# LemonATsu/DANBO-pytorch

Measured on AMD Instinct MI355X. Metric: ray-samples/sec at 512x512x64 samples, higher is better.
Workload: dtype f32 (fp16x2-split MFMA products, fp32 accumulate); 1 GPU; H36M danbo_base network, 512x512 rays x (48 coarse + 16 importance) samples, 1 pose / 1 camera per rank, cylinder near/far, exact in-volume culling; rays=262144, samples_per_ray=64, parallelism=rays-dp1

## Files before the change

danbo-pytorch_amd/csrc/common.hpp:

```cpp
#pragma once
#include <hip/hip_runtime.h>
#include <stdint.h>
#include <algorithm>
#include <atomic>
#include "../../include/danbo_hip.h"
#include "sample_math.hpp"

#define DANBO_CHECK_ARG(cond) do { if (!(cond)) return DANBO_EINVAL; } while (0)
#define DANBO_CHECK_DENSITY_ACT(act, shift) \
    DANBO_CHECK_ARG(((act) == DANBO_DENSITY_RELU || (act) == DANBO_DENSITY_SOFTPLUS) && (shift) - (shift) == 0.f)
static inline bool poses_ok(int R, int G) { return R > 0 && G > 0 && R % G == 0; }
static inline bool shape_ok(int R, int S, int G) { return S > 0 && poses_ok(R, G); }
static inline bool one_of(const void* z, const void* pts) { return (z == nullptr) != (pts == nullptr); }
#define DANBO_TRY(call) do { const int rc_ = (call); if (rc_ != 0) return rc_; } while (0)
#define DANBO_LAUNCH_RET() do { hipError_t e_ = hipGetLastError(); return e_ == hipSuccess ? 0 : (int)e_; } while (0)

#define DANBO_ENSURE_LDS(func, bytes)                                                                              \
    do {                                                                                                           \
        static std::atomic<unsigned long long> done_{0};                                                           \
        int dev_ = 0;                                                                                              \
        if (hipGetDevice(&dev_) != hipSuccess) return (int)hipGetLastError();                                      \
        const unsigned long long bit_ = 1ull << (dev_ & 63);                                                       \
        if (!(done_.load(std::memory_order_acquire) & bit_)) {                                                     \
            const hipError_t e_ = hipFuncSetAttribute(reinterpret_cast<const void*>(func),                         \
                                                      hipFuncAttributeMaxDynamicSharedMemorySize, (int)(bytes));   \
            if (e_ != hipSuccess) return (int)e_;                                                                  \
            done_.fetch_or(bit_, std::memory_order_release);                                                       \
        }                                                                                                          \
    } while (0)

#if defined(__HIP_DEVICE_COMPILE__)
#define DANBO_NO_PK_F32 __attribute__((target("no-packed-fp32-ops")))
#else
#define DANBO_NO_PK_F32
#endif

namespace danbo {

constexpr int WAVE = 64;
typedef _Float16 half8 __attribute__((ext_vector_type(8)));
typedef float f32x4 __attribute__((ext_vector_type(4)));
typedef float f32x16 __attribute__((ext_vector_type(16)));
typedef unsigned u32x4 __attribute__((ext_vector_type(4)));

#ifdef DANBO_DEV_SWITCHES
static inline int dev_env(const char* name, int dflt) { const char* e = getenv(name); return e ? atoi(e) : dflt; }
#else
static constexpr int dev_env(const char*, int dflt) { return dflt; }
#endif

static inline int num_cu() {
    static std::atomic<int> cached_[64];
    int dev = 0;
    if (hipGetDevice(&dev) != hipSuccess) return 256;
    std::atomic<int>& c = cached_[dev & 63];
    int n = c.load(std::memory_order_relaxed);
    if (n == 0) {
        if (hipDeviceGetAttribute(&n, hipDeviceAttributeMultiprocessorCount, dev) != hipSuccess || n <= 0) n = 256;
        { const int v = dev_env("DANBO_NUM_CU", 0); if (v > 0 && v <= n) n = v; }
        c.store(n, std::memory_order_relaxed);
    }
    return n;
}

struct Carver {
    char* base = nullptr;
    size_t used = 0;
    Carver() {}
    explicit Carver(void* workspace) : base(reinterpret_cast<char*>(((uintptr_t)workspace + 255) & ~(uintptr_t)255)) {}
    void align() { used = (used + 255) & ~(size_t)255; }
    template <class T>
    T* take(size_t n) {
        align();
        T* p = base ? reinterpret_cast<T*>(base + used) : nullptr;
        used += n * sizeof(T);
        return p;
    }
};

static inline int ceil_div(long a, long b) { return (int)((a + b - 1) / b); }

static inline int stream_grid(long items, int block) {
    long g = (items + block - 1) / block;
    const long cap = (long)num_cu() * 8;
    if (g > cap) g = cap;
    if (g < 1) g = 1;
    return (int)g;
}

template <class K>
static inline int resident_grid(K kernel, long items, int block, size_t lds = 0) {
    int per_cu = 0;
    if (hipOccupancyMaxActiveBlocksPerMultiprocessor(&per_cu, kernel, block, lds) != hipSuccess || per_cu < 1) per_cu = 1;
    long g = (items + block - 1) / block;
    const long cap = (long)num_cu() * per_cu;
    if (g > cap) g = cap;
    if (g < 1) g = 1;
    return (int)g;
}

__device__ __forceinline__ float wave_sum(float v) {
#pragma unroll
    for (int off = 32; off > 0; off >>= 1) v += __shfl_xor(v, off, 64);
    return v;
}

__device__ __forceinline__ void pe_sincos(float x, float* s, float* c) {
    const float k = rintf(x * 0.636619772367581343f);
    float r = fmaf(k, -1.57079601287841796875f, x);
    r = fmaf(k, -3.1391647326017846353352069854736328125e-7f, r);
    r = fmaf(k, -5.390302529957764765544681040410068817436695098876953125e-15f, r);
    const float r2 = r * r;
    float sp = fmaf(r2, 2.6083159809786593541502952575683593750e-6f, -1.981069071916863322258e-4f);
    sp = fmaf(sp, r2, 8.33307858556509017944e-3f);
    sp = fmaf(sp, r2, -1.66666597127914428711e-1f);
    const float sn = fmaf(sp * r2, r, r);
    float cp = fmaf(r2, 2.44331571593647822737693786621e-5f, -1.38873163610696792602539062500e-3f);
    cp = fmaf(cp, r2, 4.16666455566883087158203125e-2f);
    cp = fmaf(cp, r2, -0.5f);
    const float cs = fmaf(cp, r2, 1.0f);
    const int q = (int)k;
    const float s0 = (q & 1) ? cs : sn;
    const float c0 = (q & 1) ? sn : cs;
    *s = (q & 2) ? -s0 : s0;
    *c = ((q + 1) & 2) ? -c0 : c0;
}

#define DANBO_DPP_STEP(OP, IDENT, CTRL, ROWMASK)                                                              \
    {                                                                                                          \
        const int t_ = __builtin_amdgcn_update_dpp(__builtin_bit_cast(int, (float)(IDENT)),                    \
                                                   __builtin_bit_cast(int, x), CTRL, ROWMASK, 0xf, false);     \
        x = OP(x, __builtin_bit_cast(float, t_));                                                              \
    }
__device__ __forceinline__ float dpp_add_(float a, float b) { return add_rn(a, b); }
__device__ __forceinline__ float dpp_mul_(float a, float b) { return mul_rn(a, b); }

__device__ __forceinline__ float wave_scan_add(float x) {
    DANBO_DPP_STEP(dpp_add_, 0.f, 0x111, 0xf) DANBO_DPP_STEP(dpp_add_, 0.f, 0x112, 0xf)
    DANBO_DPP_STEP(dpp_add_, 0.f, 0x114, 0xf) DANBO_DPP_STEP(dpp_add_, 0.f, 0x118, 0xf)
    DANBO_DPP_STEP(dpp_add_, 0.f, 0x142, 0xa) DANBO_DPP_STEP(dpp_add_, 0.f, 0x143, 0xc)
    return x;
}
__device__ __forceinline__ float wave_scan_mul(float x) {
    DANBO_DPP_STEP(dpp_mul_, 1.f, 0x111, 0xf) DANBO_DPP_STEP(dpp_mul_, 1.f, 0x112, 0xf)
    DANBO_DPP_STEP(dpp_mul_, 1.f, 0x114, 0xf) DANBO_DPP_STEP(dpp_mul_, 1.f, 0x118, 0xf)
    DANBO_DPP_STEP(dpp_mul_, 1.f, 0x142, 0xa) DANBO_DPP_STEP(dpp_mul_, 1.f, 0x143, 0xc)
    return x;
}
__device__ __forceinline__ uint32_t wave_or(uint32_t x) {
#define DANBO_DPP_OR(CTRL, ROWMASK) x |= (uint32_t)__builtin_amdgcn_update_dpp(0, (int)x, CTRL, ROWMASK, 0xf, false);
    DANBO_DPP_OR(0x111, 0xf) DANBO_DPP_OR(0x112, 0xf) DANBO_DPP_OR(0x114, 0xf) DANBO_DPP_OR(0x118, 0xf)
    DANBO_DPP_OR(0x142, 0xa) DANBO_DPP_OR(0x143, 0xc)
#undef DANBO_DPP_OR
    return (uint32_t)__builtin_amdgcn_readlane((int)x, 63);
}
__device__ __forceinline__ float wave_total(float x) {
    return __builtin_bit_cast(float, __builtin_amdgcn_readlane(__builtin_bit_cast(int, wave_scan_add(x)), 63));
}

__device__ __forceinline__ float lane_xor32(float x) {
    const unsigned u = __builtin_bit_cast(unsigned, x);
    const auto r = __builtin_amdgcn_permlane32_swap(u, u, false, false);
    return __builtin_bit_cast(float, (threadIdx.x & 32) ? r[0] : r[1]);
}
__device__ __forceinline__ float lane_xor16(float x) {
    const unsigned u = __builtin_bit_cast(unsigned, x);
    const auto r = __builtin_amdgcn_permlane16_swap(u, u, false, false);
    return __builtin_bit_cast(float, (threadIdx.x & 16) ? r[0] : r[1]);
}

static __global__ __launch_bounds__(256) void k_zero_words_(uint32_t* __restrict__ p0, long n0, uint32_t* __restrict__ p1, long n1) {
    const long stride = (long)gridDim.x * blockDim.x;
    for (long i = (long)blockIdx.x * blockDim.x + threadIdx.x; i < n0; i += stride) p0[i] = 0u;
    for (long i = (long)blockIdx.x * blockDim.x + threadIdx.x; i < n1; i += stride) p1[i] = 0u;
}
static inline void zero_words(void* p0, long n0, void* p1, long n1, hipStream_t st) {
    const long n = n0 > n1 ? n0 : n1;
    hipLaunchKernelGGL(k_zero_words_, dim3(stream_grid(n, 256)), dim3(256), 0, st, static_cast<uint32_t*>(p0), n0,
                       static_cast<uint32_t*>(p1), p1 ? n1 : 0);
}
static __global__ __launch_bounds__(64) void k_copy_words_(const uint32_t* __restrict__ s0, uint32_t* __restrict__ d0, int n0,
                                                           const uint32_t* __restrict__ s1, uint32_t* __restrict__ d1, int n1) {
    for (int i = threadIdx.x; i < n0; i += 64) d0[i] = s0[i];
    for (int i = threadIdx.x; i < n1; i += 64) d1[i] = s1[i];
}

template <int BLOCK>
__device__ __forceinline__ void stage_bone_tables(const float* __restrict__ align, const float* __restrict__ axis_scale,
                                                  float* s_align, float* s_scale, float pad) {
    for (int i = threadIdx.x; i < J * 16; i += BLOCK) s_align[i] = align[i];
    for (int i = threadIdx.x; i < J * 4; i += BLOCK) s_scale[i] = (i & 3) < 3 ? fabsf(axis_scale[(i >> 2) * 3 + (i & 3)]) : pad;
}

__device__ __forceinline__ int resolve_count(const int32_t* count, int n_cap) {
    if (count == nullptr) return n_cap;
    int c = *count;
    return c < n_cap ? c : n_cap;
}

template <class H8>
__device__ __forceinline__ void split8_mix(const float* v, H8& hi, H8& lo) {
    u32x4 h, l;
#pragma unroll
    for (int p = 0; p < 4; ++p) {
        unsigned hp, lp;
        asm("v_cvt_pk_f16_f32 %0, %1, %2" : "=v"(hp) : "v"(v[2 * p]), "v"(v[2 * p + 1]));
        asm("v_fma_mixlo_f16 %0, %1, 1.0, -%2 op_sel:[0,0,0] op_sel_hi:[0,0,1]" : "=v"(lp) : "v"(v[2 * p]), "v"(hp));
        asm("v_fma_mixhi_f16 %0, %1, 1.0, -%2 op_sel:[0,0,1] op_sel_hi:[0,0,1]" : "+v"(lp) : "v"(v[2 * p + 1]), "v"(hp));
        h[p] = hp;
        l[p] = lp;
    }
    hi = __builtin_bit_cast(H8, h);
    lo = __builtin_bit_cast(H8, l);
}


}
```

danbo-pytorch_amd/csrc/k_sample.hip:

```cpp
#include "common.hpp"
#include "cull_math.hpp"

namespace danbo {

__global__ __launch_bounds__(256) DANBO_NO_PK_F32 void k_cylinder_pass1(const float* __restrict__ rays_o,
                                                        const float* __restrict__ rays_d,
                                                        const float* __restrict__ cyl, int R, int G,
                                                        float near0, float far0,
                                                        const float* __restrict__ near_in,
                                                        const float* __restrict__ far_in, int chunk,
                                                        double* __restrict__ acc,
                                                        float* __restrict__ near_out,
                                                        float* __restrict__ far_out) {
    const int rays_per_pose = R / G;
    for (int r0 = blockIdx.x * blockDim.x; r0 < R; r0 += gridDim.x * blockDim.x) {
        const int r = r0 + threadIdx.x;
        const bool act = r < R;
        const int rc = act ? r : R - 1;
        const int g = min(rc / rays_per_pose, G - 1);
        float o[3] = {rays_o[3 * rc], rays_o[3 * rc + 1], rays_o[3 * rc + 2]};
        float d[3] = {rays_d[3 * rc], rays_d[3 * rc + 1], rays_d[3 * rc + 2]};
        float c[3] = {cyl[5 * g], cyl[5 * g + 1], cyl[5 * g + 2]};
        float nr, fr;
        const bool hit = cylinder_bounds(o, d, c, near_in ? near_in[rc] : near0, far_in ? far_in[rc] : far0, &nr, &fr) && act;
// ... 378 lines not shown
            pa[0] = pts[3 * mac]; pa[1] = pts[3 * mac + 1]; pa[2] = pts[3 * mac + 2];
            pb[0] = pts[3 * mbc]; pb[1] = pts[3 * mbc + 1]; pb[2] = pts[3 * mbc + 2];
        } else {
            const float oa[3] = {rays_o[3 * ra], rays_o[3 * ra + 1], rays_o[3 * ra + 2]};
            const float da[3] = {rays_d[3 * ra], rays_d[3 * ra + 1], rays_d[3 * ra + 2]};
            const float ob[3] = {rays_o[3 * rb], rays_o[3 * rb + 1], rays_o[3 * rb + 2]};
            const float db[3] = {rays_d[3 * rb], rays_d[3 * rb + 1], rays_d[3 * rb + 2]};
            sample_point(oa, da, ma < M ? zreg[2 * pr] : z[M - 1], pa);
            sample_point(ob, db, mb < M ? zreg[2 * pr + 1] : z[M - 1], pb);
        }
        const int ga = pose_of(ra), gb = pose_of(rb);
        uint32_t ba = 0, bb = 0;
        uint32_t need = (1u << J) - 1u;
        if (ray_mask != nullptr) {
            need = wave_or(pre[2 * pr] | pre[2 * pr + 1]);
        } else if (prefilter) {
            uint32_t mine = s_mask[ra - r_first] | s_mask[rb - r_first];
            need = wave_or(mine);
        }
        if (__builtin_amdgcn_readfirstlane((int)__all(ga == gb))) {
            const v2f px = {pa[0], pb[0]}, py = {pa[1], pb[1]}, pz = {pa[2], pb[2]};
            const float* sk = s_skt + (ga - g0) * J * 16;
            in_volume_pk(sk, s_align, s_scale, need, px, py, pz, ba, bb);
        } else {
            const float* ska = s_skt + (ga - g0) * J * 16;
            const float* skb = s_skt + (gb - g0) * J * 16;
            for (int j = 0; j < J; ++j) {
                float pt[3];
                bone_local(ska + 16 * j, s_align + 16 * j, pa, pt);
                ba |= (in_volume(pt, s_scale + 4 * j) ? 1u : 0u) << j;
                bone_local(skb + 16 * j, s_align + 16 * j, pb, pt);
                bb |= (in_volume(pt, s_scale + 4 * j) ? 1u : 0u) << j;
            }
        }
        bits4[2 * pr] = ma < M ? ba : 0u;
        bits4[2 * pr + 1] = mb < M ? bb : 0u;
        if (ma < M) valid_bits[ma] = ba;
        if (mb < M) valid_bits[mb] = bb;
    }
    if (list != nullptr) {
        __shared__ int s_cnt[CULL_SPT * (CULL_BLOCK / 64)];
        __shared__ int s_base;
        const int wave = threadIdx.x >> 6;
        unsigned long long ball[CULL_SPT];
#pragma unroll
        for (int it = 0; it < CULL_SPT; ++it) {
            ball[it] = __ballot(bits4[it] != 0);
            if (lane == 0) s_cnt[it * (CULL_BLOCK / 64) + wave] = __popcll(ball[it]);
        }
        __syncthreads();
        if (threadIdx.x == 0) {
            int run = 0;
            for (int i = 0; i < CULL_SPT * (CULL_BLOCK / 64); ++i) { const int c = s_cnt[i]; s_cnt[i] = run; run += c; }
            s_base = run > 0 ? atomicAdd(count, run) : 0;
        }
        __syncthreads();
#pragma unroll
        for (int it = 0; it < CULL_SPT; ++it) {
            if (bits4[it] != 0) {
                const long m = base + it * CULL_BLOCK + threadIdx.x;
                list[s_base + s_cnt[it * (CULL_BLOCK / 64) + wave] + __popcll(ball[it] & ((1ull << lane) - 1ull))] = (int32_t)m;
            }
        }
    }
}

constexpr int GATHER_TS = 16;
constexpr int GATHER_BLOCK = GATHER_TS * J;

__global__ __launch_bounds__(GATHER_BLOCK) void k_bone_gather(const float* __restrict__ rays_o,
                                                              const float* __restrict__ rays_d,
                                                              const float* __restrict__ z,
                                                              const float* __restrict__ pts, int R, int S, int G,
                                                              const float* __restrict__ skts,
                                                              const float* __restrict__ align,
                                                              const float* __restrict__ axis_scale,
                                                              const float* __restrict__ volumes,
                                                              const int32_t* __restrict__ list,
                                                              const int32_t* __restrict__ count, int n_cap,
                                                              float* __restrict__ part_feat) {
    __shared__ __attribute__((aligned(16))) float s_vol[J * VOL];
    __shared__ __attribute__((aligned(16))) float s_out[GATHER_TS * J * FEAT];
    __shared__ __attribute__((aligned(16))) float s_skt[J * 16];
    __shared__ __attribute__((aligned(16))) float s_align[J * 16];
    __shared__ float s_scale[J * 4];

    const int n = resolve_count(count, n_cap);
    const int ntiles = (n + GATHER_TS - 1) / GATHER_TS;
    const long spp = (long)(R / G) * S;
    const int tid = threadIdx.x;
    const int sl = tid / J, j = tid % J;

    stage_bone_tables<GATHER_BLOCK>(align, axis_scale, s_align, s_scale, 1.f);
    int g_lds = -1;

    for (int tile = blockIdx.x; tile < ntiles; tile += gridDim.x) {
        const int row0 = tile * GATHER_TS;
        const int first = list ? list[row0] : row0;
        const int g_tile = pose_of_sample(first, spp, G);
        __syncthreads();
        if (g_tile != g_lds) {
            const float4* src = reinterpret_cast<const float4*>(volumes + (size_t)g_tile * J * VOL);
            float4* dst = reinterpret_cast<float4*>(s_vol);
            for (int i = tid; i < J * VOL / 4; i += GATHER_BLOCK) dst[i] = src[i];
            for (int i = tid; i < J * 16; i += GATHER_BLOCK) s_skt[i] = skts[(size_t)g_tile * J * 16 + i];
            g_lds = g_tile;
        }
        __syncthreads();
        const int row = row0 + sl;
        float* o_ = s_out + (sl * J + j) * FEAT;
        if (row < n) {
            const long m = list ? list[row] : row;
            const int g = pose_of_sample(m, spp, G);
            float p[3], pt[3], f[FEAT];
            point_of_sample(rays_o, rays_d, z, pts, m, S, p);
            if (g == g_lds) {
                bone_local(s_skt + 16 * j, s_align + 16 * j, p, pt);
                gather_bone_features(s_vol + j * VOL, pt, s_scale + 4 * j, f);
            } else {
                float sk[12];
                const float* src = skts + ((size_t)g * J + j) * 16;
#pragma unroll
                for (int i = 0; i < 12; ++i) sk[i] = src[i];
                bone_local(sk, s_align + 16 * j, p, pt);
                gather_bone_features(volumes + ((size_t)g * J + j) * VOL, pt, s_scale + 4 * j, f);
            }
#pragma unroll
            for (int k = 0; k < FEAT; ++k) o_[k] = f[k];
        } else {
#pragma unroll
            for (int k = 0; k < FEAT; ++k) o_[k] = 0.f;
        }
        __syncthreads();
        const int rows_here = min(GATHER_TS, n - row0);
        const int nvec = rows_here * (J * FEAT / 4);
        f32x4* dst = reinterpret_cast<f32x4*>(part_feat + (size_t)row0 * J * FEAT);
        const f32x4* src = reinterpret_cast<const f32x4*>(s_out);
        for (int i = tid; i < nvec; i += GATHER_BLOCK) __builtin_nontemporal_store(src[i], dst + i);
    }
}

__global__ __launch_bounds__(256) void k_fill_raw(const float4* __restrict__ raw_empty, int R, int S,
                                                  float4* __restrict__ raw) {
    const long M = (long)R * S;
    for (long m = (long)blockIdx.x * blockDim.x + threadIdx.x; m < M; m += (long)gridDim.x * blockDim.x)
        raw[m] = raw_empty[m / S];
}

__global__ __launch_bounds__(256) void k_merge_samples(const float* __restrict__ a, const float* __restrict__ b,
                                                       const int32_t* __restrict__ idx, int R, int S, int Sf, int C,
                                                       float* __restrict__ out) {
    const int St = S + Sf;
    const long N = (long)R * St;
    for (long i = (long)blockIdx.x * blockDim.x + threadIdx.x; i < N; i += (long)gridDim.x * blockDim.x) {
        const int r = (int)(i / St);
        const int src = min(max(idx[i], 0), St - 1);
        const float* s = src < S ? a + ((size_t)r * S + src) * C : b + ((size_t)r * Sf + (src - S)) * C;
        float* o = out + (size_t)i * C;
        if (C == 4) {
            *reinterpret_cast<float4*>(o) = *reinterpret_cast<const float4*>(s);
        } else {
            for (int c = 0; c < C; ++c) o[c] = s[c];
        }
    }
}

struct CompositeState {
    float carry, sr, sg, sb, sd, sa;
};

__device__ __forceinline__ int scattered_ray(long g, unsigned scatter, int R) {
    return (int)((unsigned long long)g * scatter % (unsigned)R);
}

template <int DA>
__device__ __forceinline__ float composite_chunk(CompositeState& st, const float4 rw, float zs, float gap, float dn,
                                                 float B, bool has_noise, float nz, bool act, int lane, float& al, float shift) {
    const float dist = mul_rn(gap, dn);
    float sig = div_rn(rw.w, B);
    if (has_noise) sig = add_rn(sig, nz);
    sig = density_act<DA>(sig, shift);
    al = sub_rn(1.0f, expf(-mul_rn(sig, dist)));
    if (!act) al = 0.f;
    const float t = act ? add_rn(sub_rn(1.0f, al), 1e-10f) : 1.0f;
    const float p = wave_scan_mul(t);
    float excl = __shfl_up(p, 1, 64);
    if (lane == 0) excl = 1.0f;
    const float T = mul_rn(st.carry, excl);
    st.carry = mul_rn(st.carry, __builtin_bit_cast(float, __builtin_amdgcn_readlane(__builtin_bit_cast(int, p), 63)));
    const float w = mul_rn(al, T);
    const float cr = rgb_of_logit(rw.x);
    const float cg = rgb_of_logit(rw.y);
    const float cb = rgb_of_logit(rw.z);
    st.sr += wave_total(w * cr);
    st.sg += wave_total(w * cg);
    st.sb += wave_total(w * cb);
    st.sd += wave_total(w * zs);
    st.sa += wave_total(w);
    return w;
}

__device__ __forceinline__ void composite_finish(const CompositeState& st, int r, float* __restrict__ rgb_map,
                                                 float* __restrict__ disp, float* __restrict__ acc_out) {
    rgb_map[3 * r] = st.sr;
    rgb_map[3 * r + 1] = st.sg;
    rgb_map[3 * r + 2] = st.sb;
    disp[r] = disp_of(st.sd, st.sa);
    acc_out[r] = fminf(st.sa, 1.0f);
}

__device__ __forceinline__ float ray_norm(const float* __restrict__ rays_d, int r) {
    const float dx = rays_d[3 * r], dy = rays_d[3 * r + 1], dz_ = rays_d[3 * r + 2];
    return norm3_torch(dx, dy, dz_);
}

template <int DA>
__global__ __launch_bounds__(256) void k_composite(const float4* __restrict__ raw, const float4* __restrict__ raw_empty,
                                                   const uint32_t* __restrict__ bits, const float* __restrict__ z,
                                                   const float* __restrict__ rays_d, int R, int S, float B, float shift,
                                                   const float* __restrict__ noise, float* __restrict__ rgb_map,
                                                   float* __restrict__ disp, float* __restrict__ acc_out,
                                                   float* __restrict__ weights, float* __restrict__ alpha_out,
                                                   const int32_t* __restrict__ ray_list, const int32_t* __restrict__ ray_count) {
    const int lane = threadIdx.x & 63;
    const int wave = (blockIdx.x * blockDim.x + threadIdx.x) >> 6;
    const int nwaves = (gridDim.x * blockDim.x) >> 6;
    const int n = ray_list ? min(max(*ray_count, 0), R) : R;
    for (int i = wave; i < n; i += nwaves) {
        const int r = ray_list ? min(max(ray_list[i], 0), R - 1) : i;
        const float dn = ray_norm(rays_d, r);
        const float4 re = bits ? raw_empty[r] : float4{0.f, 0.f, 0.f, 0.f};
        CompositeState st = {1.0f, 0.f, 0.f, 0.f, 0.f, 0.f};
        for (int c0 = 0; c0 < S; c0 += 64) {
            const int s = c0 + lane;
            const bool act = s < S;
            const size_t m = (size_t)r * S + (act ? s : S - 1);
            const float zs = z[m];
            const float gap = (s + 1 < S) ? sub_rn(z[m + 1], zs) : 1e10f;
            float4 rw = re;
            if (bits == nullptr || bits[m] != 0u) rw = raw[m];
            float al;
            const float w = composite_chunk<DA>(st, rw, zs, gap, dn, B, noise != nullptr, noise ? noise[m] : 0.f, act, lane, al, shift);
            if (act) {
                if (weights) weights[m] = w;
                if (alpha_out) alpha_out[m] = al;
            }
        }
        if (lane == 0) composite_finish(st, r, rgb_map, disp, acc_out);
    }
}

#define DANBO_MERGED_PARAMS                                                                                                      \
    const float4 *__restrict__ raw_a, const float4 *__restrict__ raw_b, const float4 *__restrict__ raw_empty,                    \
        const uint32_t *__restrict__ bits_a, const uint32_t *__restrict__ bits_b, const int32_t *__restrict__ sorted_idx,        \
        const float *__restrict__ z, const float *__restrict__ rays_d, int R, int S, int Sf, float B,                            \
        const float *__restrict__ noise, float *__restrict__ rgb_map, float *__restrict__ disp, float *__restrict__ acc_out,     \
        float *__restrict__ weights, float *__restrict__ alpha_out, float4 *__restrict__ raw_sorted,                             \
        const int32_t *__restrict__ ray_list, const int32_t *__restrict__ ray_count, unsigned scatter
__global__ __launch_bounds__(256) __attribute__((amdgpu_waves_per_eu(8, 8))) void k_composite_merged(DANBO_MERGED_PARAMS) {
    constexpr int DA = DENSITY_RELU;
    const float shift = 0.f;
#include "composite_merged_body.inc"
}
__global__ __launch_bounds__(256) __attribute__((amdgpu_waves_per_eu(8, 8))) void k_composite_merged_softplus(DANBO_MERGED_PARAMS,
                                                                                                              float shift) {
    constexpr int DA = DENSITY_SOFTPLUS;
#include "composite_merged_body.inc"
}
#undef DANBO_MERGED_PARAMS

template <bool TWO>
__global__ __launch_bounds__(64) void k_importance(const float* __restrict__ z, const float* __restrict__ weights,
                                                   int R, int S, int Sf, const float* __restrict__ u,
                                                   float* __restrict__ z_fine, float* __restrict__ z_sorted,
                                                   int32_t* __restrict__ sorted_idx) {
    for (int r = blockIdx.x * blockDim.x + threadIdx.x; r < R; r += gridDim.x * blockDim.x) {
        float* cdf = reinterpret_cast<float*>(sorted_idx + (size_t)r * (S + Sf));
        const float* zr = z + (size_t)r * S;
        float* zf = z_fine + (size_t)r * Sf;
        float* zs = z_sorted + (size_t)r * (S + Sf);
        int32_t* si = sorted_idx + (size_t)r * (S + Sf);
        importance_ray<TWO>(zr, weights + (size_t)r * S, S, Sf, u ? u + (size_t)r * Sf : nullptr, cdf, zf, zs, si);
        bool ascending = true;
        for (int i = 0; i + 1 < S; ++i) ascending = ascending && zr[i + 1] >= zr[i];
        if (u != nullptr || !ascending) {
            for (int i = 0; i < S; ++i) {
                int rank = 0;
                for (int k = 0; k < Sf; ++k) rank += zf[k] < zr[i];
                for (int q = 0; q < S; ++q) rank += sorts_before(zr[q], q, zr[i], i);
                zs[rank] = zr[i];
                si[rank] = i;
            }
            for (int k = 0; k < Sf; ++k) {
                int rank = 0;
                for (int i = 0; i < S; ++i) rank += zr[i] <= zf[k];
                for (int q = 0; q < Sf; ++q) rank += sorts_before(zf[q], q, zf[k], k);
                zs[rank] = zf[k];
                si[rank] = S + k;
            }
        }
    }
}

template <bool DET, bool TWO = false>
__device__ __forceinline__ void importance_wave(float zi, float wi, int r, int S, int Sf, const float* __restrict__ u,
                                                int lane, float* __restrict__ z_fine, float* __restrict__ z_sorted,
                                                int32_t* __restrict__ sorted_idx) {
    const int nb = S - 2, ncdf = S - 1;
    const bool cact = lane < S;
    const float w1 = __shfl_down(wi, 1, 64), w2 = __shfl_down(wi, 2, 64);
    const float z1 = __shfl_down(zi, 1, 64);
    float dw = 0.f;
    if (lane < nb) dw = pdf_weight<TWO>(wi, w1, w2);
    const float sum = wave_total(dw);
    const float inc = wave_scan_add(div_rn(dw, sum));
    float cdf = __shfl_up(inc, 1, 64);
    if (lane == 0) cdf = 0.f;
    const float bin = mul_rn(0.5f, add_rn(z1, zi));
    const bool fact = lane < Sf;
    const float uk = DET ? linspace01(fact ? lane : 0, Sf) : (fact ? u[(size_t)r * Sf + lane] : 0.f);
    int lo = 0, hi = ncdf;
#pragma unroll
    for (int it = 0; it < 7; ++it) {
        const int mid = (lo + hi) >> 1;
        const float cm = __shfl(cdf, mid < ncdf ? mid : ncdf - 1, 64);
        if (lo < hi) {
            if (cm > uk) hi = mid; else lo = mid + 1;
        }
    }
    const int below = cdf_below(lo), above = cdf_above(lo, ncdf);
    const float c0 = __shfl(cdf, below, 64), c1 = __shfl(cdf, above, 64);
    const float b0 = __shfl(bin, below, 64), b1 = __shfl(bin, above, 64);
    float denom = sub_rn(c1, c0);
    if (denom < 1e-5f) denom = 1.0f;
    const float t = div_rn(sub_rn(uk, c0), denom);
    const float zf = fact ? add_rn(b0, mul_rn(t, sub_rn(b1, b0))) : INFINITY;
    if (fact) z_fine[(size_t)r * Sf + lane] = zf;
    int rank_c = lane, rank_f = lane;
    const bool ascending = __all(!(lane < S - 1) || z1 >= zi);
    if (DET && ascending) {
        int l0 = 0, h0 = Sf, l1 = 0, h1 = S;
#pragma unroll
        for (int it = 0; it < 7; ++it) {
            const int m0 = (l0 + h0) >> 1, m1 = (l1 + h1) >> 1;
            const float f = __shfl(zf, m0 < 63 ? m0 : 63, 64);
            const float c = __shfl(zi, m1 < 63 ? m1 : 63, 64);
            if (l0 < h0) { if (f < zi) l0 = m0 + 1; else h0 = m0; }
            if (l1 < h1) { if (c <= zf) l1 = m1 + 1; else h1 = m1; }
        }
        rank_c += l0;
        rank_f += l1;
    } else {
        rank_c = 0;
        rank_f = 0;
        for (int k = 0; k < Sf; ++k) {
            const float zk = __shfl(zf, k, 64);
            rank_c += zk < zi;
            rank_f += sorts_before(zk, k, zf, lane);
        }
        if (ascending) rank_c += lane;
        for (int i = 0; i < S; ++i) {
            const float zc = __shfl(zi, i, 64);
            rank_f += zc <= zf;
            if (!ascending) rank_c += sorts_before(zc, i, zi, lane);
        }
    }
    const size_t o = (size_t)r * (S + Sf);
    if (cact) { z_sorted[o + rank_c] = zi; sorted_idx[o + rank_c] = lane; }
    if (fact) { z_sorted[o + rank_f] = zf; sorted_idx[o + rank_f] = S + lane; }
}

template <bool DET, bool TWO = false>
__global__ __launch_bounds__(256) void k_importance_wave(const float* __restrict__ z, const float* __restrict__ weights,
                                                         int R, int S, int Sf, const float* __restrict__ u,
                                                         float* __restrict__ z_fine, float* __restrict__ z_sorted,
                                                         int32_t* __restrict__ sorted_idx) {
    const int lane = threadIdx.x & 63;
    const int wave = (blockIdx.x * blockDim.x + threadIdx.x) >> 6;
    const int nwaves = (gridDim.x * blockDim.x) >> 6;
    for (int r = wave; r < R; r += nwaves) {
        const bool cact = lane < S;
        const float zi = cact ? z[(size_t)r * S + lane] : INFINITY;
        const float wi = cact ? weights[(size_t)r * S + lane] : 0.f;
        importance_wave<DET, TWO>(zi, wi, r, S, Sf, u, lane, z_fine, z_sorted, sorted_idx);
    }
}

constexpr int IMPB_MAX_S = 256;
template <bool DET, bool TWO = false>
__global__ __launch_bounds__(256) void k_importance_wave_long(const float* __restrict__ z, const float* __restrict__ weights,
                                                              int R, int S, int Sf, const float* __restrict__ u,
                                                              float* __restrict__ z_fine, float* __restrict__ z_sorted,
                                                              int32_t* __restrict__ sorted_idx, unsigned scatter,
                                                              const int32_t* __restrict__ ray_list,
                                                              const int32_t* __restrict__ ray_count) {
    __shared__ float s_all[4][3 * IMPB_MAX_S + 64];
    const int lane = threadIdx.x & 63, wv = threadIdx.x >> 6;
    float* s_z = s_all[wv];
    float* s_w = s_z + IMPB_MAX_S;
    float* s_b = s_w + IMPB_MAX_S;
    float* s_f = s_b + IMPB_MAX_S;
    const int wave = (blockIdx.x * blockDim.x + threadIdx.x) >> 6;
    const int nwaves = (gridDim.x * blockDim.x) >> 6;
    const int nb = S - 2, ncdf = S - 1;
    const int nchunk = (S + 63) >> 6;
    const int n = ray_list ? min(max(*ray_count, 0), R) : R;
    for (int i = wave; i < n; i += nwaves) {
        const int r = ray_list ? min(max(ray_list[i], 0), R - 1) : scattered_ray(i, scatter, R);
        const size_t o = (size_t)r * S;
        for (int c = 0; c < nchunk; ++c) {
            const int s0 = 64 * c + lane;
            if (s0 < S) { s_z[s0] = z[o + s0]; s_w[s0] = weights[o + s0]; }
        }
        float sum = 0.f;
        float dwv[IMPB_MAX_S / 64];
        bool asc = true;
#pragma unroll
        for (int c = 0; c < IMPB_MAX_S / 64; ++c) {
            const int s0 = 64 * c + lane;
            float dw = 0.f;
            if (c < nchunk && s0 < nb) {
                const float w0 = s_w[s0], w1 = s_w[s0 + 1], w2 = s_w[s0 + 2];
                dw = pdf_weight<TWO>(w0, w1, w2);
            }
            dwv[c] = dw;
            if (c < nchunk) {
                sum = add_rn(sum, wave_total(dw));
                if (s0 + 1 < S) {
                    const float z0 = s_z[s0], z1 = s_z[s0 + 1];
                    s_b[s0] = mul_rn(0.5f, add_rn(z1, z0));
                    asc = asc && z1 >= z0;
                }
            }
        }
        const bool ascending = __all(asc);
        float carry = 0.f;
#pragma unroll
        for (int c = 0; c < IMPB_MAX_S / 64; ++c) {
            if (c < nchunk) {
                const int s0 = 64 * c + lane;
                const float inc = add_rn(carry, wave_scan_add(div_rn(dwv[c], sum)));
                if (s0 < nb) s_w[s0 + 1] = inc;
                carry = __builtin_bit_cast(float, __builtin_amdgcn_readlane(__builtin_bit_cast(int, inc), 63));
            }
        }
        if (lane == 0) s_w[0] = 0.f;
        const bool fact = lane < Sf;
        const float uk = DET ? linspace01(fact ? lane : 0, Sf) : (fact ? u[(size_t)r * Sf + lane] : 0.f);
        int lo = 0, hi = ncdf;
#pragma unroll
        for (int it = 0; it < 9; ++it) {
            const int mid = (lo + hi) >> 1;
            const float cm = s_w[mid < ncdf ? mid : ncdf - 1];
            if (lo < hi) {
                if (cm > uk) hi = mid; else lo = mid + 1;
            }
        }
        const int below = cdf_below(lo), above = cdf_above(lo, ncdf);
        const float c0 = s_w[below], c1 = s_w[above];
        const float b0 = s_b[below], b1 = s_b[above];
        float denom = sub_rn(c1, c0);
        if (denom < 1e-5f) denom = 1.0f;
        const float t = div_rn(sub_rn(uk, c0), denom);
        const float zf = fact ? add_rn(b0, mul_rn(t, sub_rn(b1, b0))) : INFINITY;
        if (fact) z_fine[(size_t)r * Sf + lane] = zf;
        s_f[lane] = zf;
        const size_t oo = (size_t)r * (S + Sf);
        if (DET && ascending) {
            int l1 = 0, h1 = S;
#pragma unroll
            for (int it = 0; it < 9; ++it) {
                const int m1 = (l1 + h1) >> 1;
                const float cz = s_z[m1 < S ? m1 : S - 1];
                if (l1 < h1) { if (cz <= zf) l1 = m1 + 1; else h1 = m1; }
            }
            if (fact) { z_sorted[oo + lane + l1] = zf; sorted_idx[oo + lane + l1] = S + lane; }
            for (int c = 0; c < nchunk; ++c) {
                const int s0 = 64 * c + lane;
                const float zi = s_z[s0 < S ? s0 : S - 1];
                int l0 = 0, h0 = Sf;
#pragma unroll
                for (int it = 0; it < 7; ++it) {
                    const int m0 = (l0 + h0) >> 1;
                    const float fz = s_f[m0 < 63 ? m0 : 63];
                    if (l0 < h0) { if (fz < zi) l0 = m0 + 1; else h0 = m0; }
                }
                if (s0 < S) { z_sorted[oo + s0 + l0] = zi; sorted_idx[oo + s0 + l0] = s0; }
            }
        } else {
            int rank_f = 0;
            for (int k = 0; k < Sf; ++k) {
                const float zk = s_f[k];
                rank_f += (zk < zf) || (zk == zf && k < lane);
            }
            for (int q = 0; q < S; ++q) rank_f += s_z[q] <= zf;
            if (fact) { z_sorted[oo + rank_f] = zf; sorted_idx[oo + rank_f] = S + lane; }
            for (int c = 0; c < nchunk; ++c) {
                const int s0 = 64 * c + lane;
                const float zi = s_z[s0 < S ? s0 : S - 1];
                int rank_c = 0;
                for (int k = 0; k < Sf; ++k) rank_c += s_f[k] < zi;
                if (ascending) rank_c += s0;
                else
                    for (int q = 0; q < S; ++q) { const float zq = s_z[q]; rank_c += (zq < zi) || (zq == zi && q < s0); }
                if (s0 < S) { z_sorted[oo + rank_c] = zi; sorted_idx[oo + rank_c] = s0; }
            }
        }
    }
}

template <bool DET, bool TWO = false, int DA = DENSITY_RELU>
__global__ __launch_bounds__(256) __attribute__((amdgpu_waves_per_eu(8, 8))) void k_composite_importance(const float4* __restrict__ raw,
                                                              const float4* __restrict__ raw_empty,
                                                              const uint32_t* __restrict__ bits,
                                                              const float* __restrict__ z, const float* __restrict__ rays_d,
                                                              int R, int S, int Sf, float B, const float* __restrict__ noise,
                                                              const float* __restrict__ u, float* __restrict__ rgb_map,
                                                              float* __restrict__ disp, float* __restrict__ acc_out,
                                                              float* __restrict__ weights, float* __restrict__ alpha_out,
                                                              float* __restrict__ z_fine, float* __restrict__ z_sorted,
                                                              int32_t* __restrict__ sorted_idx,
                                                              const int32_t* __restrict__ ray_list,
                                                              const int32_t* __restrict__ ray_count, unsigned scatter, float shift) {
    const int lane = threadIdx.x & 63;
    const int wave = (blockIdx.x * blockDim.x + threadIdx.x) >> 6;
    const int nwaves = (gridDim.x * blockDim.x) >> 6;
    const bool act = lane < S;
    struct RayIn { uint32_t word; float zs, z1, dn; float4 re; };
    auto fetch = [&](int r) {
        RayIn in;
        const size_t m = (size_t)r * S + (act ? lane : S - 1);
        in.word = bits ? bits[m] : 1u;
        in.zs = z[m];
        in.z1 = (lane + 1 < S) ? z[m + 1] : 0.f;
        in.dn = ray_norm(rays_d, r);
        in.re = bits ? raw_empty[r] : float4{0.f, 0.f, 0.f, 0.f};
        return in;
    };
    const int n = ray_list ? min(max(*ray_count, 0), R) : R;
    auto ray_at = [&](int i) { return i < n ? (ray_list ? min(max(ray_list[i], 0), R - 1) : scattered_ray(i, scatter, R)) : -1; };
    int r = ray_at(wave), r_nxt = ray_at(wave + nwaves);
    if (r < 0) return;
    RayIn cur = fetch(r);
    for (int i = wave; i < n; i += nwaves) {
        CompositeState st = {1.0f, 0.f, 0.f, 0.f, 0.f, 0.f};
        const size_t m = (size_t)r * S + (act ? lane : S - 1);
        float4 rw = cur.re;
        if (cur.word != 0u) rw = raw[m];
        const int r_n = r_nxt >= 0 ? r_nxt : r;
        const RayIn nxt = fetch(r_n);
        const int r_nn = ray_at(i + 2 * nwaves);
        const float zs = cur.zs;
        const float gap = (lane + 1 < S) ? sub_rn(cur.z1, zs) : 1e10f;
        float al, w;
        bool flat = false;
        if constexpr (DA == DENSITY_RELU) {
            const float dist = mul_rn(gap, cur.dn);
            const float rgb_sum = add_rn(add_rn(cur.re.x, cur.re.y), cur.re.z);
            flat = bits != nullptr && noise == nullptr && !(div_rn(cur.re.w, B) > 0.f) && sub_rn(rgb_sum, rgb_sum) == 0.f &&
                   __all(cur.word == 0u && sub_rn(dist, dist) == 0.f);
        }
        if (flat) {
            al = 0.f;
            w = 0.f;
            st.sr = st.sg = st.sb = st.sd = st.sa = 0.f;
        } else {
            w = composite_chunk<DA>(st, rw, zs, gap, cur.dn, B, noise != nullptr, noise ? noise[m] : 0.f, act, lane, al, shift);
        }
        if (act) {
            if (weights) weights[m] = w;
            if (alpha_out) alpha_out[m] = al;
        }
        if (lane == 0) composite_finish(st, r, rgb_map, disp, acc_out);
        importance_wave<DET, TWO>(act ? zs : INFINITY, act ? w : 0.f, r, S, Sf, u, lane, z_fine, z_sorted, sorted_idx);
        cur = nxt; r = r_n; r_nxt = r_nn;
    }
}

constexpr int FLAT_BLOCK = 256;
__global__ __launch_bounds__(FLAT_BLOCK) void k_flat_rays(const float* __restrict__ t_lo,
                                                          const uint32_t* __restrict__ ray_flat, int R, int S, int Sf,
                                                          float* __restrict__ rgb0, float* __restrict__ disp0, float* __restrict__ acc0,
                                                          float* __restrict__ weights0, float* __restrict__ alpha0,
                                                          float* __restrict__ z_fine, float* __restrict__ rgb_map,
                                                          float* __restrict__ disp, float* __restrict__ acc_out,
                                                          float* __restrict__ weights, float* __restrict__ alpha_out,
                                                          int32_t* __restrict__ ray_list, int32_t* __restrict__ ray_count,
                                                          int parts) {
    __shared__ int s_cnt[FLAT_BLOCK / 64];
    __shared__ int s_base;
    const int lane = threadIdx.x & 63, wave = threadIdx.x >> 6;
    const int St = S + Sf;
    const int r = blockIdx.x * FLAT_BLOCK + threadIdx.x;
    const bool flat = r < R && ray_flat[r] != 0u;
    const float lo = flat ? t_lo[r] : 0.f;
    if (flat && (parts & 1)) {
        rgb0[3 * r] = 0.f; rgb0[3 * r + 1] = 0.f; rgb0[3 * r + 2] = 0.f;
        disp0[r] = 0.f;
        acc0[r] = 0.f;
        rgb_map[3 * r] = 0.f; rgb_map[3 * r + 1] = 0.f; rgb_map[3 * r + 2] = 0.f;
        disp[r] = 0.f;
        acc_out[r] = 0.f;
    }
    unsigned long long rows = (parts & 2) ? __ballot(flat) : 0ull;
    const unsigned long long listed = __ballot(r < R && !flat);
    while (rows != 0ull) {
        const int b = (int)__builtin_ctzll(rows);
        rows &= rows - 1ull;
        const size_t rr = (size_t)(blockIdx.x * FLAT_BLOCK + wave * 64 + b);
        for (int c = lane; c < S; c += 64) {
            if (weights0) weights0[rr * S + c] = 0.f;
            if (alpha0) alpha0[rr * S + c] = 0.f;
        }
        const float lo_b = __builtin_bit_cast(float, __builtin_amdgcn_readlane(__builtin_bit_cast(int, lo), b));
        for (int c = lane; c < Sf; c += 64) z_fine[rr * Sf + c] = lo_b;
        for (int c = lane; c < St; c += 64) {
            if (weights) weights[rr * St + c] = 0.f;
            if (alpha_out) alpha_out[rr * St + c] = 0.f;
        }
    }
    if (!(parts & 1)) return;
    if (lane == 0) s_cnt[wave] = (int)__popcll(listed);
    __syncthreads();
    if (threadIdx.x == 0) {
        int run = 0;
        for (int w = 0; w < FLAT_BLOCK / 64; ++w) { const int c = s_cnt[w]; s_cnt[w] = run; run += c; }
        s_base = run > 0 ? atomicAdd(ray_count, run) : 0;
    }
    __syncthreads();
    if (r < R && !flat) ray_list[s_base + s_cnt[wave] + (int)__popcll(listed & ((1ull << lane) - 1ull))] = r;
}

}

using namespace danbo;

static unsigned ray_scatter(int R) {
    static const unsigned primes[] = {40507u, 40519u, 40529u, 40531u, 40543u, 40559u};
    for (unsigned p : primes) {
        unsigned a = p, b = (unsigned)R;
        while (b != 0u) { const unsigned t = a % b; a = b; b = t; }
        if (a == 1u) return p;
    }
    return 1u;
}

extern "C" int danbo_near_far_cylinder(const float* rays_o, const float* rays_d, const float* cyl, int R, int G,
                                        float near0, float far0, const float* near_in, const float* far_in, int chunk,
                                        float* scratch, float* near_out, float* far_out, void* stream) {
    DANBO_CHECK_ARG(chunk > 0 && scratch != nullptr && poses_ok(R, G));
    hipStream_t st = (hipStream_t)stream;
    const int nchunk = ceil_div(R, chunk);
    if (chunk <= CYL_FUSED_MAX) {
        hipLaunchKernelGGL(k_cylinder_chunk, dim3(nchunk), dim3(CYL_BLOCK), 0, st, rays_o, rays_d, cyl, R, G, near0, far0, near_in,
                           far_in, chunk, near_out, far_out);
        DANBO_LAUNCH_RET();
    }
    zero_words(scratch, 8L * nchunk, nullptr, 0, st);
    const int grid = stream_grid(R, 256);
    hipLaunchKernelGGL(k_cylinder_pass1, dim3(grid), dim3(256), 0, st, rays_o, rays_d, cyl, R, G, near0, far0, near_in,
                       far_in, chunk, reinterpret_cast<double*>(scratch), near_out, far_out);
    hipLaunchKernelGGL(k_cylinder_pass2, dim3(grid), dim3(256), 0, st, R, near0, far0, near_in, far_in, chunk,
                       reinterpret_cast<const double*>(scratch), near_out, far_out);
    DANBO_LAUNCH_RET();
}
// ... 297 lines not shown
```

Measured before the change: 4.028 billion ray-samples/s.

## Replace shuffle-based binary searches in importance sampling with ballot counting

Swaps the per-lane binary search over the CDF, and the merge-rank binary searches, for counting formulations. Each fine sample value is broadcast with readlane and compared across the wave, a ballot popcount gives the count, and writelane places it in the owning lane. It also replaces shfl_down/shfl_up with DPP row shifts and uses readlane broadcasts in the fallback loop. The goal is to avoid the ds_bpermute LDS round trips in the shuffles, at the cost of a serial loop of scalar operations that scales with Sf. It also depends on lane_next and lane_prev shifting correctly across row boundaries, since DPP row_shr/row_shl only move data within 16-lane rows.

```diff
diff --git a/danbo-pytorch_amd/csrc/common.hpp b/danbo-pytorch_amd/csrc/common.hpp
--- a/danbo-pytorch_amd/csrc/common.hpp
+++ b/danbo-pytorch_amd/csrc/common.hpp
@@ -158,6 +158,21 @@
     return __builtin_bit_cast(float, __builtin_amdgcn_readlane(__builtin_bit_cast(int, wave_scan_add(x)), 63));
 }
 
+__device__ __forceinline__ float lane_read(float x, int k) {
+    return __builtin_bit_cast(float, __builtin_amdgcn_readlane(__builtin_bit_cast(int, x), k));
+}
+extern "C" __device__ int danbo_llvm_writelane(int v, int k, int x) __asm("llvm.amdgcn.writelane.i32");
+__device__ __forceinline__ int lane_write(int x, int k, int v) { return danbo_llvm_writelane(v, k, x); }
+__device__ __forceinline__ int wave_count(bool p) { return __builtin_popcountll(__builtin_amdgcn_ballot_w64(p)); }
+__device__ __forceinline__ float lane_next(float x) {
+    const int u = __builtin_bit_cast(int, x);
+    return __builtin_bit_cast(float, __builtin_amdgcn_update_dpp(u, u, 0x130, 0xf, 0xf, false));
+}
+__device__ __forceinline__ float lane_prev(float x, float first) {
+    return __builtin_bit_cast(float, __builtin_amdgcn_update_dpp(__builtin_bit_cast(int, first), __builtin_bit_cast(int, x), 0x138,
+                                                                 0xf, 0xf, false));
+}
+
 __device__ __forceinline__ float lane_xor32(float x) {
     const unsigned u = __builtin_bit_cast(unsigned, x);
     const auto r = __builtin_amdgcn_permlane32_swap(u, u, false, false);
diff --git a/danbo-pytorch_amd/csrc/k_sample.hip b/danbo-pytorch_amd/csrc/k_sample.hip
--- a/danbo-pytorch_amd/csrc/k_sample.hip
+++ b/danbo-pytorch_amd/csrc/k_sample.hip
@@ -704,32 +704,46 @@
     }
 }
 
+template <int K0, class F>
+__device__ __forceinline__ void fine_samples_by4(int n, F&& f) {
+    if constexpr (K0 < 64) {
+        if (K0 < n) {
+            f(K0);
+            fine_samples_by4<K0 + 4>(n, f);
+        }
+    }
+}
+
 template <bool DET, bool TWO = false>
 __device__ __forceinline__ void importance_wave(float zi, float wi, int r, int S, int Sf, const float* __restrict__ u,
                                                 int lane, float* __restrict__ z_fine, float* __restrict__ z_sorted,
                                                 int32_t* __restrict__ sorted_idx) {
     const int nb = S - 2, ncdf = S - 1;
     const bool cact = lane < S;
-    const float w1 = __shfl_down(wi, 1, 64), w2 = __shfl_down(wi, 2, 64);
-    const float z1 = __shfl_down(zi, 1, 64);
+    const float w1 = lane_next(wi), w2 = lane_next(w1);
+    const float z1 = lane_next(zi);
     float dw = 0.f;
     if (lane < nb) dw = pdf_weight<TWO>(wi, w1, w2);
     const float sum = wave_total(dw);
     const float inc = wave_scan_add(div_rn(dw, sum));
-    float cdf = __shfl_up(inc, 1, 64);
-    if (lane == 0) cdf = 0.f;
+    const float cdf = lane_prev(inc, 0.f);
     const float bin = mul_rn(0.5f, add_rn(z1, zi));
     const bool fact = lane < Sf;
     const float uk = DET ? linspace01(fact ? lane : 0, Sf) : (fact ? u[(size_t)r * Sf + lane] : 0.f);
-    int lo = 0, hi = ncdf;
-#pragma unroll
-    for (int it = 0; it < 7; ++it) {
-        const int mid = (lo + hi) >> 1;
-        const float cm = __shfl(cdf, mid < ncdf ? mid : ncdf - 1, 64);
-        if (lo < hi) {
-            if (cm > uk) hi = mid; else lo = mid + 1;
-        }
-    }
+    int lo = 0;
+    const float cdf_in = lane < ncdf ? cdf : NAN;
+    int n_fine = Sf;
+    asm volatile("" : "+s"(n_fine));
+    fine_samples_by4<0>(n_fine, [&](int k0) {
+        float u_k[4];
+        int n_k[4];
+#pragma unroll
+        for (int j = 0; j < 4; ++j) u_k[j] = lane_read(uk, k0 + j);
+#pragma unroll
+        for (int j = 0; j < 4; ++j) n_k[j] = wave_count(cdf_in <= u_k[j]);
+#pragma unroll
+        for (int j = 0; j < 4; ++j) lo = lane_write(lo, k0 + j, n_k[j]);
+    });
     const int below = cdf_below(lo), above = cdf_above(lo, ncdf);
     const float c0 = __shfl(cdf, below, 64), c1 = __shfl(cdf, above, 64);
     const float b0 = __shfl(bin, below, 64), b1 = __shfl(bin, above, 64);
@@ -741,28 +755,32 @@
     int rank_c = lane, rank_f = lane;
     const bool ascending = __all(!(lane < S - 1) || z1 >= zi);
     if (DET && ascending) {
-        int l0 = 0, h0 = Sf, l1 = 0, h1 = S;
-#pragma unroll
-        for (int it = 0; it < 7; ++it) {
-            const int m0 = (l0 + h0) >> 1, m1 = (l1 + h1) >> 1;
-            const float f = __shfl(zf, m0 < 63 ? m0 : 63, 64);
-            const float c = __shfl(zi, m1 < 63 ? m1 : 63, 64);
-            if (l0 < h0) { if (f < zi) l0 = m0 + 1; else h0 = m0; }
-            if (l1 < h1) { if (c <= zf) l1 = m1 + 1; else h1 = m1; }
-        }
-        rank_c += l0;
-        rank_f += l1;
+        const float z_in = cact ? zi : NAN;
+        int before = 0;
+        fine_samples_by4<0>(n_fine, [&](int k0) {
+            float zk[4];
+            int n_k[4];
+#pragma unroll
+            for (int j = 0; j < 4; ++j) zk[j] = lane_read(zf, k0 + j);
+#pragma unroll
+            for (int j = 0; j < 4; ++j) n_k[j] = wave_count(z_in <= zk[j]);
+#pragma unroll
+            for (int j = 0; j < 4; ++j) before = lane_write(before, k0 + j, n_k[j]);
+#pragma unroll
+            for (int j = 0; j < 4; ++j) rank_c += zk[j] < z_in;
+        });
+        rank_f += before;
     } else {
         rank_c = 0;
         rank_f = 0;
         for (int k = 0; k < Sf; ++k) {
-            const float zk = __shfl(zf, k, 64);
+            const float zk = lane_read(zf, k);
             rank_c += zk < zi;
             rank_f += sorts_before(zk, k, zf, lane);
         }
         if (ascending) rank_c += lane;
         for (int i = 0; i < S; ++i) {
-            const float zc = __shfl(zi, i, 64);
+            const float zc = lane_read(zi, i);
             rank_f += zc <= zf;
             if (!ascending) rank_c += sorts_before(zc, i, zi, lane);
         }
```

Result: no change. 4.041 billion ray-samples/s (median of 6 runs) (+0.3%).
